# facebookresearch/nonrigid_nerf

Hardware: NVIDIA H100
Metric: rays/sec (64c+128f samples, 8x256 MLP), example_sequence training step (higher is better)
Workload: dtype f16 (tensor-core operands; f32 accumulate)

## Files before the change

### __graft_entry__.py

```python
import os
import subprocess
import sys

ROOT = os.path.dirname(os.path.abspath(__file__))
if ROOT not in sys.path:
    sys.path.insert(0, ROOT)


def build() -> None:
    subprocess.check_call(["make", "-j", str(min(8, os.cpu_count() or 1)), "-C", os.path.join(ROOT, "nonrigid_nerf_b200", "csrc")])
    subprocess.check_call(["make", "-C", os.path.join(ROOT, "tests", "cuda")])
    subprocess.check_call(["make", "-C", os.path.join(ROOT, "tests", "cuda"), "-f", "wgmma_rs_probe.mk"])
    import nonrigid_nerf_b200
    from nonrigid_nerf_b200 import _lib

    lib = _lib.load()
    assert lib.nrn_abi_version() == _lib.ABI_VERSION
    import oracle.nrnerf_oracle
    subprocess.check_call([sys.executable, os.path.join(ROOT, "oracle", "make_ref.py")])


def smoke() -> None:
    import numpy as np
    import torch

    import oracle.nrnerf_oracle as O
    from nonrigid_nerf_b200 import _lib, train as T
    from tests import helpers

    dev = "cuda:0"
    seed, n = 4242, 96
    coarse, fine, bender, (cp, fp, bp) = helpers.build_models(O, seed, dev)
    r = O.make_rays(seed, n)
    rnd = O.make_randomness(seed, n, 64, 64)
    lat = r["latents"].clone().to(dev).requires_grad_(True)
    kw = dict(network_query_fn=None, perturb=1.0, N_importance=64, network_fine=fine, N_samples=64, network_fn=coarse,
              ray_bender=bender, use_viewdirs=False, white_bkgd=False, raw_noise_std=1.0, ndc=False, lindisp=False,
              randomness=rnd)
    rgb, disp, acc, extras = T.render(r["rays_o"].to(dev), r["rays_d"].to(dev), chunk=32768, near=r["near"], far=r["far"],
                                      additional_pixel_information={"ray_bending_latents": lat}, detailed_output=True,
                                      retraw=True, **kw)
    tgt = r["target"].to(dev)
    loss = ((rgb - tgt) ** 2).mean() + ((extras["rgb0"] - tgt) ** 2).mean()
    loss.backward()
    _lib.device_error_check()

    cpo, fpo, bpo = O.clone_params(cp, True), O.clone_params(fp, True), O.clone_params(bp, True)
    ret = O.render_rays(cpo, fpo, bpo, r["rays_o"], r["rays_d"], r["near"], r["far"], r["latents"], 64, 64, perturb=True,
                        raw_noise_std=1.0, rnd=rnd)
    (((ret["rgb_map"] - r["target"]) ** 2).mean() + ((ret["rgb0"] - r["target"]) ** 2).mean()).backward()
    linf = float((rgb.detach().cpu() - ret["rgb_map"].detach()).abs().max())
    g, g_ref = fine.pts_linears[3].weight.grad.cpu(), fpo["pts_w"][3].grad
    rel = float((g - g_ref).norm() / g_ref.norm())
    print(f"smoke: rgb L-inf vs oracle {linf:.3e}; grad rel err (fine L3) {rel:.3e}; loss {float(loss):.5f}")
    assert np.isfinite(float(loss)) and linf <= 5e-4 and rel <= 3e-2, (linf, rel)


if __name__ == "__main__":
    build()
    if len(sys.argv) > 1 and sys.argv[1] == "smoke":
        smoke()
```

### nonrigid_nerf_b200/csrc/field_bwd.cu

```cuda
#include "field_mma.cuh"

namespace nrn {

namespace {

constexpr int kBwdStageLd = 66;
constexpr int kBwdRingStages = 4;
constexpr size_t kBwdSmemBytes = kHBytes + kBwdRingStages * kRingStageBytes + 2 * kWgRows * kBwdStageLd * sizeof(float) +
                                 sizeof(RingShared<kBwdRingStages>) + 64;
static_assert(kBwdSmemBytes <= 227 * 1024, "DGRAD kernel: dynamic shared memory per block");

static_assert(dgrad::step(dgrad::L6T) == dgrad::step(dgrad::L7T) && dgrad::step(dgrad::L5hT) == dgrad::step(dgrad::L7T) &&
              dgrad::step(dgrad::L4T) == dgrad::step(dgrad::L7T) && dgrad::step(dgrad::L3T) == dgrad::step(dgrad::L7T) &&
              dgrad::step(dgrad::L2T) == dgrad::step(dgrad::L7T) && dgrad::step(dgrad::L1T) == dgrad::step(dgrad::L7T),
              "step_at: one default shape; the consumers run L5h^T .. L1^T as one loop");
constexpr uint32_t kSlabA = 2 * dgrad::step(dgrad::L4T).k16 * kChunkBytes;

__device__ __forceinline__ Step step_at(int step) {
  switch (step) {
    case dgrad::HeadT: return step_imm<dgrad::HeadT>();
    case dgrad::L5eT: return step_imm<dgrad::L5eT>();
    case dgrad::L0T: return step_imm<dgrad::L0T>();
    case dgrad::B4T: return step_imm<dgrad::B4T>();
    case dgrad::B3T: return step_imm<dgrad::B3T>();
    case dgrad::B2T: return step_imm<dgrad::B2T>();
    case dgrad::B1T: return step_imm<dgrad::B1T>();
    case dgrad::B0T: return step_imm<dgrad::B0T>();
    default: return step_imm<dgrad::L7T>();
  }
}

__device__ __forceinline__ float clamp_h(float v) { return fminf(fmaxf(v, -65504.f), 65504.f); }

template <int NCOLS, int NR>
__device__ __forceinline__ void epi_mask_store(const float (&acc)[NR], const ReluMask<NCOLS>& m, uint8_t* img, int g) {
  const int r0 = g * kWgRows + acc_r0(), q = acc_q();
#pragma unroll
  for (int j = 0; j < NCOLS / 8; ++j) {
#pragma unroll
    for (int i = 0; i < 2; ++i) {
      const uint32_t g2 = pack_h2_sat(acc[4 * j + 2 * i], acc[4 * j + 2 * i + 1]);
      *reinterpret_cast<uint32_t*>(img + j * kChunkBytes + (r0 + 8 * i) * 16 + 4 * q) = m.apply(i, j, g2);
    }
  }
}

__device__ __forceinline__ float h_lo(uint32_t w) { return __half2float(__ushort_as_half(static_cast<unsigned short>(w & 0xffffu))); }
__device__ __forceinline__ float h_hi(uint32_t w) { return __half2float(__ushort_as_half(static_cast<unsigned short>(w >> 16))); }

__device__ __forceinline__ void pe_backward(const float* de, const uint8_t* __restrict__ e_row, float (&dx)[3]) {
  float e[64];
#pragma unroll
  for (int c = 0; c < 8; ++c) {
    const uint4 w = __ldg(reinterpret_cast<const uint4*>(e_row + c * kChunkBytes));
    e[c * 8 + 0] = h_lo(w.x); e[c * 8 + 1] = h_hi(w.x); e[c * 8 + 2] = h_lo(w.y); e[c * 8 + 3] = h_hi(w.y);
    e[c * 8 + 4] = h_lo(w.z); e[c * 8 + 5] = h_hi(w.z); e[c * 8 + 6] = h_lo(w.w); e[c * 8 + 7] = h_hi(w.w);
  }
#pragma unroll
  for (int d = 0; d < 3; ++d) {
    float acc = de[d];
#pragma unroll
    for (int k = 0; k < 10; ++k) {
      const float f = static_cast<float>(1 << k);
      const float s = e[3 + 6 * k + d], c = e[3 + 6 * k + 3 + d];
      acc += f * (de[3 + 6 * k + d] * c - de[3 + 6 * k + 3 + d] * s);
    }
    dx[d] += acc;
  }
}

}

template <bool HAS_BENDER>
__global__ void __launch_bounds__(kFwdThreads, 1) field_bwd_kernel(const FieldBwdParams p) {
  extern __shared__ __align__(1024) uint8_t smem[];
  uint8_t* act = smem;
  uint8_t* ring_buf = smem + kHBytes;
  float* stage_all = reinterpret_cast<float*>(ring_buf + kBwdRingStages * kRingStageBytes);
  auto* sh = reinterpret_cast<RingShared<kBwdRingStages>*>(stage_all + 2 * kWgRows * kBwdStageLd);

  const int warp = threadIdx.x >> 5;
  const int lane = threadIdx.x & 31;

  if (threadIdx.x == 0) sh->init();
  __syncthreads();
  const Waiter W{&sh->abort_flag, p.err};
  Ring<kBwdRingStages> ring{ring_buf, sh->w_full, sh->w_empty};

  if (warp >= 8) {
    setmaxnreg_dec<kProducerRegs>();
    if (warp == 8 && lane == 0) produce(p.nerf_wT, p.bend_wT, p.n_tiles, 0, HAS_BENDER ? dgrad::kCount : dgrad::B4T, dgrad::B4T, step_at, ring, W);
    return;
  }

  setmaxnreg_inc<kConsumerRegs>();
  const int g = warp >> 2;
  const int tw = threadIdx.x & 127;
  const bool row_thread = tw < kWgRows;
  const int bar = 1 + g;
  const bool wg_leader = tw == 0;
  const int row = g * kWgRows + tw;
  uint8_t* a_row = act + row * 16;
  const uint32_t a_base = smem_u32(act) + g * kWgRows * 16;
  auto a_slab = [&](uint32_t j) { return a_base + j * kSlabA; };
  float* stg = stage_all + g * kWgRows * kBwdStageLd;
  const float* my_stg = stg + tw * kBwdStageLd;

  const float scale = loss_scale(p.amax);
  const float inv_scale = 1.0f / scale;

  for (int tile = blockIdx.x; tile < p.n_tiles; tile += gridDim.x) {
    const long long pt = static_cast<long long>(tile) * kTileM + row;
    const bool valid = row_thread && pt < p.P;
    const uint8_t* st_tile = p.stash + static_cast<long long>(tile) * kStashTileBytes;
    const uint8_t* st = st_tile + row * 16;
    uint8_t* gs = p.gstash + static_cast<long long>(tile) * kGradTileBytes;
    const StashWriter<false> sw{gs, wg_leader, bar, g};
    const uint8_t* mk = p.relu_mask + static_cast<long long>(tile) * kMaskTileBytes;
    auto prefetch_e = [&]() {
      if (wg_leader) tma_prefetch_l2(st_tile + kStE.off, kEBytes);
    };
    sw.begin();
    if (row_thread) {
      float gr[4] = {0.f, 0.f, 0.f, 0.f};
      if (valid) {
        const float* q = p.d_raw + pt * p.out_ch;
#pragma unroll
        for (int c = 0; c < 4; ++c) gr[c] = clamp_h(__ldg(q + c) * scale);
      }
      *reinterpret_cast<uint4*>(a_row) = make_uint4(pack_h2(gr[0], gr[1]), pack_h2(gr[2], gr[3]), 0u, 0u);
      *reinterpret_cast<uint4*>(a_row + kChunkBytes) = make_uint4(0u, 0u, 0u, 0u);
    }
    sw.ready(kGsRaw, act);
    float dx[3] = {0.f, 0.f, 0.f};
#pragma unroll 1
    for (int s = 0; s < 3; ++s) {
      const Step st = step_at(dgrad::HeadT + s);
      Acc<dgrad::L7T> acc;
      ReluMask<kMaskHCols> m;
      m.load(mk + kMkH + (7 - s) * kMaskHBytes, g);
      wg_gemm<dgrad::step(dgrad::L7T).N>(acc, ring, st.nslabs, st.k16, a_slab, W, 300 + s);
      if (s == 2) prefetch_e();
      sw.begin();
      epi_mask_store<kMaskHCols>(acc, m, act, g);
      sw.ready({kGsY + (7 - s) * kHBytes, kHChunks}, act);
    }
    {
      Acc<dgrad::L5eT> acc;
      wg_gemm_step<dgrad::L5eT>(acc, ring, a_slab, W, 303);
      stage_cols<0, 8>(acc, stg, kBwdStageLd);
      wg_bar(bar);
      if (row_thread) pe_backward(my_stg, st + kStE.off, dx);
    }
#pragma unroll 1
    for (int s = 0; s < 5; ++s) {
      Acc<dgrad::L4T> acc;
      ReluMask<kMaskHCols> m;
      m.load(mk + kMkH + (4 - s) * kMaskHBytes, g);
      wg_gemm_step<dgrad::L4T>(acc, ring, a_slab, W, 304 + s);
      if (s == 4) prefetch_e();
      sw.begin();
      epi_mask_store<kMaskHCols>(acc, m, act, g);
      sw.ready({kGsY + (4 - s) * kHBytes, kHChunks}, act);
    }
    {
      Acc<dgrad::L0T> acc;
      wg_gemm_step<dgrad::L0T>(acc, ring, a_slab, W, 309);
      stage_cols<0, 8>(acc, stg, kBwdStageLd);
      wg_bar(bar);
      if (row_thread) pe_backward(my_stg, st + kStE.off, dx);
    }
    if (!HAS_BENDER) continue;

    float drpre = 0.f;
    sw.begin();
    if (row_thread) {
      float rig = 0.f, un[3] = {0.f, 0.f, 0.f}, dun[3], dm[3];
      float up_r = 0.f, up_u[3] = {0.f, 0.f, 0.f};
      if (valid) {
        rig = __ldg(p.rigidity + pt);
#pragma unroll
        for (int d = 0; d < 3; ++d) un[d] = __ldg(p.unmasked + pt * 3 + d);
        if (p.d_rigid_up) up_r = __ldg(p.d_rigid_up + pt) * scale;
        if (p.d_unmasked_up) {
#pragma unroll
          for (int d = 0; d < 3; ++d) up_u[d] = __ldg(p.d_unmasked_up + pt * 3 + d) * scale;
        }
      }
      float dr = up_r;
#pragma unroll
      for (int d = 0; d < 3; ++d) {
        dm[d] = p.use_scaling ? dx[d] * p.scaling : dx[d];
        dun[d] = rig * dm[d] + up_u[d];
        dr += un[d] * dm[d];
      }
      drpre = dr * 2.0f * rig * (1.0f - rig);
      if (p.use_cutoff && rig <= p.cutoff) drpre = 0.f;
      if (!valid) { dun[0] = dun[1] = dun[2] = 0.f; drpre = 0.f; }
      *reinterpret_cast<uint4*>(a_row) = make_uint4(pack_h2(clamp_h(dun[0]), clamp_h(dun[1])), pack_h2(clamp_h(dun[2]), 0.f), 0u, 0u);
      *reinterpret_cast<uint4*>(a_row + kChunkBytes) = make_uint4(0u, 0u, 0u, 0u);
    }
    sw.ready(kGsYb4, act);
    {
      Acc<dgrad::B4T> acc;
      ReluMask<kMkHb4.cols> m;
      m.load(mk + kMkHb4.off, g);
      wg_gemm_step<dgrad::B4T>(acc, ring, a_slab, W, 310);
      sw.begin();
      epi_mask_store<kMkHb4.cols>(acc, m, act, g);
      sw.ready(kGsYb3, act);
    }
    {
      Acc<dgrad::B3T> acc;
      ReluMask<kMkHb3.cols> m;
      m.load(mk + kMkHb3.off, g);
      wg_gemm_step<dgrad::B3T>(acc, ring, a_slab, W, 311);
      sw.begin();
      epi_mask_store<kMkHb3.cols>(acc, m, act, g);
      if (row_thread) {
        *reinterpret_cast<uint4*>(a_row + 8 * kChunkBytes) = make_uint4(pack_h2(clamp_h(drpre), 0.f), 0u, 0u, 0u);
        *reinterpret_cast<uint4*>(a_row + 9 * kChunkBytes) = make_uint4(0u, 0u, 0u, 0u);
      }
      sw.ready(kGsYb2, act);
    }
    {
      Acc<dgrad::B2T> acc;
      ReluMask<kMkHb2.cols> m;
      m.load(mk + kMkHb2.off, g);
      wg_gemm_step<dgrad::B2T>(acc, ring, a_slab, W, 312);
      sw.begin();
      epi_mask_store<kMkHb2.cols>(acc, m, act, g);
      sw.ready(kGsYb1, act);
      m.load(mk + kMkHb1.off, g);
      wg_gemm_step<dgrad::B1T>(acc, ring, a_slab, W, 313);
      sw.begin();
      epi_mask_store<kMkHb1.cols>(acc, m, act, g);
      sw.ready(kGsYb0, act);
    }
    {
      Acc<dgrad::B0T> acc;
      wg_gemm_step<dgrad::B0T>(acc, ring, a_slab, W, 314);
      stage_cols<0, 5>(acc, stg, kBwdStageLd);
      wg_bar(bar);
      if (row_thread) {
        float dl[32];
#pragma unroll
        for (int i = 0; i < 32; ++i) dl[i] = my_stg[6 + i] * inv_scale;
        const long long ray = valid ? pt / p.S : -1;
        const long long ray0 = __shfl_sync(0xffffffffu, ray, 0);
        if (__all_sync(0xffffffffu, ray == ray0 && valid)) {
          const float tot = warp_transpose_reduce(dl, lane);
          atomicAdd(p.d_latents + ray0 * kLatent + lane, tot);
        } else if (valid) {
#pragma unroll
          for (int i = 0; i < 32; ++i) atomicAdd(p.d_latents + ray * kLatent + i, dl[i]);
        }
      }
    }
  }
  if (wg_leader) tma_bulk_wait<0>();
}

cudaError_t launch_field_bwd(const FieldBwdParams& p, bool has_bender, int num_sms, cudaStream_t stream) {
  return launch_field(has_bender ? field_bwd_kernel<true> : field_bwd_kernel<false>, p, num_sms, kBwdSmemBytes, stream);
}

}
```

### nonrigid_nerf_b200/csrc/sm90_ptx.cuh

```cuda
#pragma once
#include <cuda_runtime.h>
#include <cuda_fp16.h>
#include <cuda_bf16.h>
#include <stdint.h>

namespace nrn {

__device__ __forceinline__ uint32_t smem_u32(const void* p) {
  return static_cast<uint32_t>(__cvta_generic_to_shared(p));
}

__device__ __forceinline__ void mbar_init(uint64_t* bar, uint32_t count) {
  asm volatile("mbarrier.init.shared::cta.b64 [%0], %1;\n" ::"r"(smem_u32(bar)), "r"(count) : "memory");
}
__device__ __forceinline__ void fence_mbar_init() {
  asm volatile("fence.mbarrier_init.release.cluster;\n" ::: "memory");
}
__device__ __forceinline__ void mbar_arrive(uint64_t* bar) {
  asm volatile("mbarrier.arrive.shared::cta.b64 _, [%0];\n" ::"r"(smem_u32(bar)) : "memory");
}
__device__ __forceinline__ void mbar_arrive_expect_tx(uint64_t* bar, uint32_t bytes) {
  asm volatile("mbarrier.arrive.expect_tx.shared::cta.b64 _, [%0], %1;\n" ::"r"(smem_u32(bar)), "r"(bytes)
               : "memory");
}
__device__ __forceinline__ bool mbar_try_wait(uint64_t* bar, uint32_t parity) {
  uint32_t ok;
  asm volatile(
      "{\n\t.reg .pred P;\n\t"
      "mbarrier.try_wait.parity.shared::cta.b64 P, [%1], %2;\n\t"
      "selp.b32 %0, 1, 0, P;\n\t}\n"
      : "=r"(ok)
      : "r"(smem_u32(bar)), "r"(parity)
      : "memory");
  return ok != 0;
}

__device__ __forceinline__ uint32_t cluster_ctarank() {
  uint32_t r;
  asm volatile("mov.u32 %0, %%cluster_ctarank;\n" : "=r"(r));
  return r;
}
__device__ __forceinline__ void cluster_sync() {
  asm volatile("barrier.cluster.arrive.release.aligned;\n\tbarrier.cluster.wait.acquire.aligned;\n" ::: "memory");
}
__device__ __forceinline__ uint32_t mapa_shared(const void* p, uint32_t rank) {
  uint32_t r;
  asm volatile("mapa.shared::cluster.u32 %0, %1, %2;\n" : "=r"(r) : "r"(smem_u32(p)), "r"(rank));
  return r;
}
__device__ __forceinline__ void mbar_arrive_cluster(uint32_t cluster_addr) {
  asm volatile("mbarrier.arrive.shared::cluster.b64 _, [%0];\n" ::"r"(cluster_addr) : "memory");
}
__device__ __forceinline__ void st_shared_cluster(uint32_t cluster_addr, int v) {
  asm volatile("st.relaxed.cluster.shared::cluster.u32 [%0], %1;\n" ::"r"(cluster_addr), "r"(v) : "memory");
}

__device__ __forceinline__ void fence_proxy_async_smem() {
  asm volatile("fence.proxy.async.shared::cta;\n" ::: "memory");
}

__device__ __forceinline__ void wg_bar(int id) { asm volatile("bar.sync %0, 128;" ::"r"(id) : "memory"); }

__device__ __forceinline__ void tma_bulk_g2s(void* smem_dst, const void* gmem_src, uint32_t bytes,
                                             uint64_t* bar) {
  asm volatile(
      "cp.async.bulk.shared::cluster.global.mbarrier::complete_tx::bytes [%0], [%1], %2, [%3];\n" ::"r"(
          smem_u32(smem_dst)),
      "l"(gmem_src), "r"(bytes), "r"(smem_u32(bar))
      : "memory");
}
__device__ __forceinline__ void tma_bulk_g2s_multicast(void* smem_dst, const void* gmem_src, uint32_t bytes, uint64_t* bar,
                                                       uint16_t cta_mask) {
  asm volatile(
      "cp.async.bulk.shared::cluster.global.mbarrier::complete_tx::bytes.multicast::cluster [%0], [%1], %2, [%3], %4;\n" ::"r"(
          smem_u32(smem_dst)),
      "l"(gmem_src), "r"(bytes), "r"(smem_u32(bar)), "h"(cta_mask)
      : "memory");
}
__device__ __forceinline__ void tma_bulk_s2g(void* gmem_dst, const void* smem_src, uint32_t bytes) {
  asm volatile("cp.async.bulk.global.shared::cta.bulk_group [%0], [%1], %2;\n" ::"l"(gmem_dst),
               "r"(smem_u32(smem_src)), "r"(bytes)
               : "memory");
}
__device__ __forceinline__ void tma_prefetch_l2(const void* gmem_src, uint32_t bytes) {
  asm volatile("cp.async.bulk.prefetch.L2.global [%0], %1;\n" ::"l"(gmem_src), "r"(bytes) : "memory");
}
__device__ __forceinline__ void tma_bulk_commit() { asm volatile("cp.async.bulk.commit_group;\n" ::: "memory"); }
template <int N>
__device__ __forceinline__ void tma_bulk_wait_read() {
  asm volatile("cp.async.bulk.wait_group.read %0;\n" ::"n"(N) : "memory");
}
template <int N>
__device__ __forceinline__ void tma_bulk_wait() {
  asm volatile("cp.async.bulk.wait_group %0;\n" ::"n"(N) : "memory");
}

template <int R>
__device__ __forceinline__ void setmaxnreg_dec() { asm volatile("setmaxnreg.dec.sync.aligned.u32 %0;\n" ::"n"(R)); }
template <int R>
__device__ __forceinline__ void setmaxnreg_inc() { asm volatile("setmaxnreg.inc.sync.aligned.u32 %0;\n" ::"n"(R)); }

__host__ __device__ __forceinline__ uint64_t gmma_desc(uint32_t saddr, uint32_t lbo_bytes, uint32_t sbo_bytes) {
  uint64_t d = 0;
  d |= static_cast<uint64_t>((saddr >> 4) & 0x3FFFu);
  d |= static_cast<uint64_t>((lbo_bytes >> 4) & 0x3FFFu) << 16;
  d |= static_cast<uint64_t>((sbo_bytes >> 4) & 0x3FFFu) << 32;
  return d;
}
__host__ __device__ __forceinline__ uint64_t gmma_desc_advance(uint64_t desc, uint32_t bytes) {
  return desc + static_cast<uint64_t>(bytes >> 4);
}

__device__ __forceinline__ void wgmma_fence() { asm volatile("wgmma.fence.sync.aligned;\n" ::: "memory"); }
__device__ __forceinline__ void wgmma_commit() { asm volatile("wgmma.commit_group.sync.aligned;\n" ::: "memory"); }
template <int NR>
__device__ __forceinline__ void acc_fence(float (&d)[NR]) {
#pragma unroll
  for (int i = 0; i < NR; ++i) asm volatile("" : "+f"(d[i])::"memory");
}
template <int N>
__device__ __forceinline__ void wgmma_wait() {
  asm volatile("wgmma.wait_group.sync.aligned %0;\n" ::"n"(N) : "memory");
}

template <int TA, int TB>
__device__ __forceinline__ void wgmma_m64n16(float (&d)[8], uint64_t adesc, uint64_t bdesc, uint32_t accumulate) {
  asm volatile(
      "{\n\t.reg .pred p;\n\t"
      "setp.ne.b32 p, %10, 0;\n\t"
      "wgmma.mma_async.sync.aligned.m64n16k16.f32.f16.f16 "
      "{%0, %1, %2, %3, %4, %5, %6, %7}, "
      "%8, %9, p, 1, 1, %11, %12;\n\t}\n"
      : "+f"(d[0]), "+f"(d[1]), "+f"(d[2]), "+f"(d[3]), "+f"(d[4]), "+f"(d[5]), "+f"(d[6]), "+f"(d[7])
      : "l"(adesc), "l"(bdesc), "r"(accumulate), "n"(TA), "n"(TB));
}

template <int TA, int TB>
__device__ __forceinline__ void wgmma_m64n48(float (&d)[24], uint64_t adesc, uint64_t bdesc, uint32_t accumulate) {
  asm volatile(
      "{\n\t.reg .pred p;\n\t"
      "setp.ne.b32 p, %26, 0;\n\t"
      "wgmma.mma_async.sync.aligned.m64n48k16.f32.f16.f16 "
      "{%0, %1, %2, %3, %4, %5, %6, %7, %8, %9, %10, %11, %12, %13, %14, %15, %16, %17, %18, %19, %20, %21, %22, %23}, "
      "%24, %25, p, 1, 1, %27, %28;\n\t}\n"
      : "+f"(d[0]), "+f"(d[1]), "+f"(d[2]), "+f"(d[3]), "+f"(d[4]), "+f"(d[5]), "+f"(d[6]), "+f"(d[7]), "+f"(d[8]), "+f"(d[9]), "+f"(d[10]), "+f"(d[11]), "+f"(d[12]), "+f"(d[13]), "+f"(d[14]), "+f"(d[15]), "+f"(d[16]), "+f"(d[17]), "+f"(d[18]), "+f"(d[19]), "+f"(d[20]), "+f"(d[21]), "+f"(d[22]), "+f"(d[23])
      : "l"(adesc), "l"(bdesc), "r"(accumulate), "n"(TA), "n"(TB));
}

template <int TA, int TB>
__device__ __forceinline__ void wgmma_m64n64(float (&d)[32], uint64_t adesc, uint64_t bdesc, uint32_t accumulate) {
  asm volatile(
      "{\n\t.reg .pred p;\n\t"
      "setp.ne.b32 p, %34, 0;\n\t"
      "wgmma.mma_async.sync.aligned.m64n64k16.f32.f16.f16 "
      "{%0, %1, %2, %3, %4, %5, %6, %7, %8, %9, %10, %11, %12, %13, %14, %15, %16, %17, %18, %19, %20, %21, %22, %23, %24, %25, %26, %27, %28, %29, %30, %31}, "
      "%32, %33, p, 1, 1, %35, %36;\n\t}\n"
      : "+f"(d[0]), "+f"(d[1]), "+f"(d[2]), "+f"(d[3]), "+f"(d[4]), "+f"(d[5]), "+f"(d[6]), "+f"(d[7]), "+f"(d[8]), "+f"(d[9]), "+f"(d[10]), "+f"(d[11]), "+f"(d[12]), "+f"(d[13]), "+f"(d[14]), "+f"(d[15]), "+f"(d[16]), "+f"(d[17]), "+f"(d[18]), "+f"(d[19]), "+f"(d[20]), "+f"(d[21]), "+f"(d[22]), "+f"(d[23]), "+f"(d[24]), "+f"(d[25]), "+f"(d[26]), "+f"(d[27]), "+f"(d[28]), "+f"(d[29]), "+f"(d[30]), "+f"(d[31])
      : "l"(adesc), "l"(bdesc), "r"(accumulate), "n"(TA), "n"(TB));
}

template <int TA, int TB>
__device__ __forceinline__ void wgmma_m64n80(float (&d)[40], uint64_t adesc, uint64_t bdesc, uint32_t accumulate) {
  asm volatile(
      "{\n\t.reg .pred p;\n\t"
      "setp.ne.b32 p, %42, 0;\n\t"
      "wgmma.mma_async.sync.aligned.m64n80k16.f32.f16.f16 "
      "{%0, %1, %2, %3, %4, %5, %6, %7, %8, %9, %10, %11, %12, %13, %14, %15, %16, %17, %18, %19, %20, %21, %22, %23, %24, %25, %26, %27, %28, %29, %30, %31, %32, %33, %34, %35, %36, %37, %38, %39}, "
      "%40, %41, p, 1, 1, %43, %44;\n\t}\n"
      : "+f"(d[0]), "+f"(d[1]), "+f"(d[2]), "+f"(d[3]), "+f"(d[4]), "+f"(d[5]), "+f"(d[6]), "+f"(d[7]), "+f"(d[8]), "+f"(d[9]), "+f"(d[10]), "+f"(d[11]), "+f"(d[12]), "+f"(d[13]), "+f"(d[14]), "+f"(d[15]), "+f"(d[16]), "+f"(d[17]), "+f"(d[18]), "+f"(d[19]), "+f"(d[20]), "+f"(d[21]), "+f"(d[22]), "+f"(d[23]), "+f"(d[24]), "+f"(d[25]), "+f"(d[26]), "+f"(d[27]), "+f"(d[28]), "+f"(d[29]), "+f"(d[30]), "+f"(d[31]), "+f"(d[32]), "+f"(d[33]), "+f"(d[34]), "+f"(d[35]), "+f"(d[36]), "+f"(d[37]), "+f"(d[38]), "+f"(d[39])
      : "l"(adesc), "l"(bdesc), "r"(accumulate), "n"(TA), "n"(TB));
}

template <int TA, int TB>
__device__ __forceinline__ void wgmma_m64n96(float (&d)[48], uint64_t adesc, uint64_t bdesc, uint32_t accumulate) {
  asm volatile(
      "{\n\t.reg .pred p;\n\t"
      "setp.ne.b32 p, %50, 0;\n\t"
      "wgmma.mma_async.sync.aligned.m64n96k16.f32.f16.f16 "
      "{%0, %1, %2, %3, %4, %5, %6, %7, %8, %9, %10, %11, %12, %13, %14, %15, %16, %17, %18, %19, %20, %21, %22, %23, %24, %25, %26, %27, %28, %29, %30, %31, %32, %33, %34, %35, %36, %37, %38, %39, %40, %41, %42, %43, %44, %45, %46, %47}, "
      "%48, %49, p, 1, 1, %51, %52;\n\t}\n"
      : "+f"(d[0]), "+f"(d[1]), "+f"(d[2]), "+f"(d[3]), "+f"(d[4]), "+f"(d[5]), "+f"(d[6]), "+f"(d[7]), "+f"(d[8]), "+f"(d[9]), "+f"(d[10]), "+f"(d[11]), "+f"(d[12]), "+f"(d[13]), "+f"(d[14]), "+f"(d[15]), "+f"(d[16]), "+f"(d[17]), "+f"(d[18]), "+f"(d[19]), "+f"(d[20]), "+f"(d[21]), "+f"(d[22]), "+f"(d[23]), "+f"(d[24]), "+f"(d[25]), "+f"(d[26]), "+f"(d[27]), "+f"(d[28]), "+f"(d[29]), "+f"(d[30]), "+f"(d[31]), "+f"(d[32]), "+f"(d[33]), "+f"(d[34]), "+f"(d[35]), "+f"(d[36]), "+f"(d[37]), "+f"(d[38]), "+f"(d[39]), "+f"(d[40]), "+f"(d[41]), "+f"(d[42]), "+f"(d[43]), "+f"(d[44]), "+f"(d[45]), "+f"(d[46]), "+f"(d[47])
      : "l"(adesc), "l"(bdesc), "r"(accumulate), "n"(TA), "n"(TB));
}

template <int TA, int TB>
__device__ __forceinline__ void wgmma_m64n256(float (&d)[128], uint64_t adesc, uint64_t bdesc, uint32_t accumulate) {
  asm volatile(
      "{\n\t.reg .pred p;\n\t"
      "setp.ne.b32 p, %130, 0;\n\t"
      "wgmma.mma_async.sync.aligned.m64n256k16.f32.f16.f16 "
      "{%0, %1, %2, %3, %4, %5, %6, %7, %8, %9, %10, %11, %12, %13, %14, %15, %16, %17, %18, %19, %20, %21, %22, %23, %24, %25, %26, %27, %28, %29, %30, %31, %32, %33, %34, %35, %36, %37, %38, %39, %40, %41, %42, %43, %44, %45, %46, %47, %48, %49, %50, %51, %52, %53, %54, %55, %56, %57, %58, %59, %60, %61, %62, %63, %64, %65, %66, %67, %68, %69, %70, %71, %72, %73, %74, %75, %76, %77, %78, %79, %80, %81, %82, %83, %84, %85, %86, %87, %88, %89, %90, %91, %92, %93, %94, %95, %96, %97, %98, %99, %100, %101, %102, %103, %104, %105, %106, %107, %108, %109, %110, %111, %112, %113, %114, %115, %116, %117, %118, %119, %120, %121, %122, %123, %124, %125, %126, %127}, "
      "%128, %129, p, 1, 1, %131, %132;\n\t}\n"
      : "+f"(d[0]), "+f"(d[1]), "+f"(d[2]), "+f"(d[3]), "+f"(d[4]), "+f"(d[5]), "+f"(d[6]), "+f"(d[7]), "+f"(d[8]), "+f"(d[9]), "+f"(d[10]), "+f"(d[11]), "+f"(d[12]), "+f"(d[13]), "+f"(d[14]), "+f"(d[15]), "+f"(d[16]), "+f"(d[17]), "+f"(d[18]), "+f"(d[19]), "+f"(d[20]), "+f"(d[21]), "+f"(d[22]), "+f"(d[23]), "+f"(d[24]), "+f"(d[25]), "+f"(d[26]), "+f"(d[27]), "+f"(d[28]), "+f"(d[29]), "+f"(d[30]), "+f"(d[31]), "+f"(d[32]), "+f"(d[33]), "+f"(d[34]), "+f"(d[35]), "+f"(d[36]), "+f"(d[37]), "+f"(d[38]), "+f"(d[39]), "+f"(d[40]), "+f"(d[41]), "+f"(d[42]), "+f"(d[43]), "+f"(d[44]), "+f"(d[45]), "+f"(d[46]), "+f"(d[47]), "+f"(d[48]), "+f"(d[49]), "+f"(d[50]), "+f"(d[51]), "+f"(d[52]), "+f"(d[53]), "+f"(d[54]), "+f"(d[55]), "+f"(d[56]), "+f"(d[57]), "+f"(d[58]), "+f"(d[59]), "+f"(d[60]), "+f"(d[61]), "+f"(d[62]), "+f"(d[63]), "+f"(d[64]), "+f"(d[65]), "+f"(d[66]), "+f"(d[67]), "+f"(d[68]), "+f"(d[69]), "+f"(d[70]), "+f"(d[71]), "+f"(d[72]), "+f"(d[73]), "+f"(d[74]), "+f"(d[75]), "+f"(d[76]), "+f"(d[77]), "+f"(d[78]), "+f"(d[79]), "+f"(d[80]), "+f"(d[81]), "+f"(d[82]), "+f"(d[83]), "+f"(d[84]), "+f"(d[85]), "+f"(d[86]), "+f"(d[87]), "+f"(d[88]), "+f"(d[89]), "+f"(d[90]), "+f"(d[91]), "+f"(d[92]), "+f"(d[93]), "+f"(d[94]), "+f"(d[95]), "+f"(d[96]), "+f"(d[97]), "+f"(d[98]), "+f"(d[99]), "+f"(d[100]), "+f"(d[101]), "+f"(d[102]), "+f"(d[103]), "+f"(d[104]), "+f"(d[105]), "+f"(d[106]), "+f"(d[107]), "+f"(d[108]), "+f"(d[109]), "+f"(d[110]), "+f"(d[111]), "+f"(d[112]), "+f"(d[113]), "+f"(d[114]), "+f"(d[115]), "+f"(d[116]), "+f"(d[117]), "+f"(d[118]), "+f"(d[119]), "+f"(d[120]), "+f"(d[121]), "+f"(d[122]), "+f"(d[123]), "+f"(d[124]), "+f"(d[125]), "+f"(d[126]), "+f"(d[127])
      : "l"(adesc), "l"(bdesc), "r"(accumulate), "n"(TA), "n"(TB));
}

template <int N, int TA, int TB>
__device__ __forceinline__ void wgmma(float (&d)[N / 2], uint64_t adesc, uint64_t bdesc, uint32_t accumulate) {
  static_assert(N == 16 || N == 48 || N == 64 || N == 80 || N == 96 || N == 256, "wgmma: N without a wrapper");
  if constexpr (N == 16) wgmma_m64n16<TA, TB>(d, adesc, bdesc, accumulate);
  else if constexpr (N == 48) wgmma_m64n48<TA, TB>(d, adesc, bdesc, accumulate);
  else if constexpr (N == 64) wgmma_m64n64<TA, TB>(d, adesc, bdesc, accumulate);
  else if constexpr (N == 80) wgmma_m64n80<TA, TB>(d, adesc, bdesc, accumulate);
  else if constexpr (N == 96) wgmma_m64n96<TA, TB>(d, adesc, bdesc, accumulate);
  else wgmma_m64n256<TA, TB>(d, adesc, bdesc, accumulate);
}

template <int TB>
__device__ __forceinline__ void wgmma_m64n16_rs(float (&d)[8], const uint32_t (&a)[4], uint64_t bdesc, uint32_t accumulate) {
  asm volatile(
      "{\n\t.reg .pred p;\n\t"
      "setp.ne.b32 p, %13, 0;\n\t"
      "wgmma.mma_async.sync.aligned.m64n16k16.f32.f16.f16 "
      "{%0, %1, %2, %3, %4, %5, %6, %7}, "
      "{%8, %9, %10, %11}, %12, p, 1, 1, %14;\n\t}\n"
      : "+f"(d[0]), "+f"(d[1]), "+f"(d[2]), "+f"(d[3]), "+f"(d[4]), "+f"(d[5]), "+f"(d[6]), "+f"(d[7])
      : "r"(a[0]), "r"(a[1]), "r"(a[2]), "r"(a[3]), "l"(bdesc), "r"(accumulate), "n"(TB));
}

template <int TB>
__device__ __forceinline__ void wgmma_m64n256_rs(float (&d)[128], const uint32_t (&a)[4], uint64_t bdesc, uint32_t accumulate) {
  asm volatile(
      "{\n\t.reg .pred p;\n\t"
      "setp.ne.b32 p, %133, 0;\n\t"
      "wgmma.mma_async.sync.aligned.m64n256k16.f32.f16.f16 "
      "{%0, %1, %2, %3, %4, %5, %6, %7, %8, %9, %10, %11, %12, %13, %14, %15, %16, %17, %18, %19, %20, %21, %22, %23, %24, %25, %26, %27, %28, %29, %30, %31, %32, %33, %34, %35, %36, %37, %38, %39, %40, %41, %42, %43, %44, %45, %46, %47, %48, %49, %50, %51, %52, %53, %54, %55, %56, %57, %58, %59, %60, %61, %62, %63, %64, %65, %66, %67, %68, %69, %70, %71, %72, %73, %74, %75, %76, %77, %78, %79, %80, %81, %82, %83, %84, %85, %86, %87, %88, %89, %90, %91, %92, %93, %94, %95, %96, %97, %98, %99, %100, %101, %102, %103, %104, %105, %106, %107, %108, %109, %110, %111, %112, %113, %114, %115, %116, %117, %118, %119, %120, %121, %122, %123, %124, %125, %126, %127}, "
      "{%128, %129, %130, %131}, %132, p, 1, 1, %134;\n\t}\n"
      : "+f"(d[0]), "+f"(d[1]), "+f"(d[2]), "+f"(d[3]), "+f"(d[4]), "+f"(d[5]), "+f"(d[6]), "+f"(d[7]), "+f"(d[8]), "+f"(d[9]), "+f"(d[10]), "+f"(d[11]), "+f"(d[12]), "+f"(d[13]), "+f"(d[14]), "+f"(d[15]), "+f"(d[16]), "+f"(d[17]), "+f"(d[18]), "+f"(d[19]), "+f"(d[20]), "+f"(d[21]), "+f"(d[22]), "+f"(d[23]), "+f"(d[24]), "+f"(d[25]), "+f"(d[26]), "+f"(d[27]), "+f"(d[28]), "+f"(d[29]), "+f"(d[30]), "+f"(d[31]), "+f"(d[32]), "+f"(d[33]), "+f"(d[34]), "+f"(d[35]), "+f"(d[36]), "+f"(d[37]), "+f"(d[38]), "+f"(d[39]), "+f"(d[40]), "+f"(d[41]), "+f"(d[42]), "+f"(d[43]), "+f"(d[44]), "+f"(d[45]), "+f"(d[46]), "+f"(d[47]), "+f"(d[48]), "+f"(d[49]), "+f"(d[50]), "+f"(d[51]), "+f"(d[52]), "+f"(d[53]), "+f"(d[54]), "+f"(d[55]), "+f"(d[56]), "+f"(d[57]), "+f"(d[58]), "+f"(d[59]), "+f"(d[60]), "+f"(d[61]), "+f"(d[62]), "+f"(d[63]), "+f"(d[64]), "+f"(d[65]), "+f"(d[66]), "+f"(d[67]), "+f"(d[68]), "+f"(d[69]), "+f"(d[70]), "+f"(d[71]), "+f"(d[72]), "+f"(d[73]), "+f"(d[74]), "+f"(d[75]), "+f"(d[76]), "+f"(d[77]), "+f"(d[78]), "+f"(d[79]), "+f"(d[80]), "+f"(d[81]), "+f"(d[82]), "+f"(d[83]), "+f"(d[84]), "+f"(d[85]), "+f"(d[86]), "+f"(d[87]), "+f"(d[88]), "+f"(d[89]), "+f"(d[90]), "+f"(d[91]), "+f"(d[92]), "+f"(d[93]), "+f"(d[94]), "+f"(d[95]), "+f"(d[96]), "+f"(d[97]), "+f"(d[98]), "+f"(d[99]), "+f"(d[100]), "+f"(d[101]), "+f"(d[102]), "+f"(d[103]), "+f"(d[104]), "+f"(d[105]), "+f"(d[106]), "+f"(d[107]), "+f"(d[108]), "+f"(d[109]), "+f"(d[110]), "+f"(d[111]), "+f"(d[112]), "+f"(d[113]), "+f"(d[114]), "+f"(d[115]), "+f"(d[116]), "+f"(d[117]), "+f"(d[118]), "+f"(d[119]), "+f"(d[120]), "+f"(d[121]), "+f"(d[122]), "+f"(d[123]), "+f"(d[124]), "+f"(d[125]), "+f"(d[126]), "+f"(d[127])
      : "r"(a[0]), "r"(a[1]), "r"(a[2]), "r"(a[3]), "l"(bdesc), "r"(accumulate), "n"(TB));
}

template <int N, int TB>
__device__ __forceinline__ void wgmma_rs(float (&d)[N / 2], const uint32_t (&a)[4], uint64_t bdesc, uint32_t accumulate) {
  static_assert(N == 16 || N == 256, "wgmma_rs: N without a wrapper");
  if constexpr (N == 16) wgmma_m64n16_rs<TB>(d, a, bdesc, accumulate);
  else wgmma_m64n256_rs<TB>(d, a, bdesc, accumulate);
}
template <int KF>
__device__ __forceinline__ uint32_t& frag_pair(uint32_t (&a)[KF][4], int j, int i) { return a[j >> 1][2 * (j & 1) + i]; }
template <int KF>
__device__ __forceinline__ void frag_fence(uint32_t (&a)[KF][4]) {
#pragma unroll
  for (int k = 0; k < KF; ++k)
#pragma unroll
    for (int i = 0; i < 4; ++i) asm volatile("" : "+r"(a[k][i])::"memory");
}

__device__ __forceinline__ uint32_t pack_h2(float a, float b) {
  __half2 h = __floats2half2_rn(a, b);
  return *reinterpret_cast<uint32_t*>(&h);
}
__device__ __forceinline__ uint32_t pack_h2_relu_sat(float a, float b) {
  uint32_t d;
  asm("cvt.rn.relu.satfinite.f16x2.f32 %0, %1, %2;" : "=r"(d) : "f"(b), "f"(a));
  return d;
}
__device__ __forceinline__ uint32_t pack_h2_sat(float a, float b) {
  uint32_t d;
  asm("cvt.rn.satfinite.f16x2.f32 %0, %1, %2;" : "=r"(d) : "f"(b), "f"(a));
  return d;
}
__device__ __forceinline__ uint32_t pack_bf2(float a, float b) {
  __nv_bfloat162 h = __floats2bfloat162_rn(a, b);
  return *reinterpret_cast<uint32_t*>(&h);
}

constexpr long long kWaitLimitCycles = 1ll << 28;

struct Waiter {
  int* s_abort;
  int* g_err;
  bool paired = false;
  uint32_t partner_abort = 0;
  __device__ __forceinline__ bool wait(uint64_t* bar, uint32_t parity, int code) const {
    if (mbar_try_wait(bar, parity)) return true;
    const long long t0 = clock64();
    while (!mbar_try_wait(bar, parity)) {
      if (*reinterpret_cast<volatile int*>(s_abort)) return false;
      if (clock64() - t0 > kWaitLimitCycles) {
        atomicExch(s_abort, code);
        if (paired) st_shared_cluster(partner_abort, code);
        atomicCAS(g_err, 0, code);
        return false;
      }
    }
    return true;
  }
};

template <int N>
__device__ __forceinline__ void transpose_reduce_step(float (&v)[32], int lane) {
  if constexpr (N > 1) {
    constexpr int off = N / 2;
    const bool upper = (lane & off) != 0;
#pragma unroll
    for (int i = 0; i < off; ++i) {
      const float lo = v[i], hi = v[i + off];
      v[i] = (upper ? hi : lo) + __shfl_xor_sync(0xffffffffu, upper ? lo : hi, off);
    }
    transpose_reduce_step<off>(v, lane);
  }
}

__device__ __forceinline__ float warp_transpose_reduce(float (&v)[32], int lane) {
  transpose_reduce_step<32>(v, lane);
  return v[0];
}

__device__ __forceinline__ float loss_scale(const float* amax_ptr) {
  float scale = 1.0f;
  const float amax = amax_ptr ? __ldg(amax_ptr) : 0.f;
  if (amax > 0.f && amax < 3.0e38f) {
    int e;
    frexpf(amax, &e);
    scale = ldexpf(1.0f, min(max(10 - e, -60), 60));
  }
  return scale;
}

}
```

Before: 424,100.

## Keep dgrad trunk activations in registers via wgmma RS operand, add ring stage

The backward dgrad trunk (head^T through L0^T) now feeds the next layer's MMA straight from register fragments (wgmma with A from registers) instead of writing the masked gradient to a shared activation slab and reading it back through descriptors. Gradient images still go to global scratch for the weight-gradient pass. The freed shared-memory activation area shrinks to the bender image size, which allows one more weight ring stage. A new m64n64 RS wrapper is added for the embedding-sized steps. The cost is much higher register pressure (128 accumulators plus 64 fragment registers per thread) and extra warpgroup barriers around staging.

After: 454,600 (median of 6 runs). +7.2%, better.

```diff
diff --git a/__graft_entry__.py b/__graft_entry__.py
--- a/__graft_entry__.py
+++ b/__graft_entry__.py
@@ -11,6 +11,7 @@
     subprocess.check_call(["make", "-j", str(min(8, os.cpu_count() or 1)), "-C", os.path.join(ROOT, "nonrigid_nerf_b200", "csrc")])
     subprocess.check_call(["make", "-C", os.path.join(ROOT, "tests", "cuda")])
     subprocess.check_call(["make", "-C", os.path.join(ROOT, "tests", "cuda"), "-f", "wgmma_rs_probe.mk"])
+    subprocess.check_call(["make", "-C", os.path.join(ROOT, "tests", "cuda"), "-f", "wgmma_rs64_probe.mk"])
     import nonrigid_nerf_b200
     from nonrigid_nerf_b200 import _lib
 
diff --git a/nonrigid_nerf_b200/csrc/field_bwd.cu b/nonrigid_nerf_b200/csrc/field_bwd.cu
--- a/nonrigid_nerf_b200/csrc/field_bwd.cu
+++ b/nonrigid_nerf_b200/csrc/field_bwd.cu
@@ -5,8 +5,11 @@
 namespace {
 
 constexpr int kBwdStageLd = 66;
-constexpr int kBwdRingStages = 4;
-constexpr size_t kBwdSmemBytes = kHBytes + kBwdRingStages * kRingStageBytes + 2 * kWgRows * kBwdStageLd * sizeof(float) +
+constexpr int kBwdActBytes = kGsYb1.chunks * kChunkBytes;
+static_assert(kGsYb4.chunks <= kGsYb1.chunks && kGsYb3.chunks <= kGsYb1.chunks && kGsYb2.chunks <= kGsYb1.chunks &&
+              kGsYb0.chunks <= kGsYb1.chunks, "bender gradient images fit act");
+constexpr int kBwdRingStages = 5;
+constexpr size_t kBwdSmemBytes = kBwdActBytes + kBwdRingStages * kRingStageBytes + 2 * kWgRows * kBwdStageLd * sizeof(float) +
                                  sizeof(RingShared<kBwdRingStages>) + 64;
 static_assert(kBwdSmemBytes <= 227 * 1024, "DGRAD kernel: dynamic shared memory per block");
 
@@ -45,6 +48,20 @@
   }
 }
 
+__device__ __forceinline__ void epi_mask_frag(const float (&acc)[kMaskHCols / 2], const ReluMask<kMaskHCols>& m,
+                                              uint32_t (&a)[kMaskHCols / 16][4], uint8_t* gs_img, int g) {
+  const int r0 = g * kWgRows + acc_r0(), q = acc_q();
+#pragma unroll
+  for (int j = 0; j < kMaskHCols / 8; ++j) {
+#pragma unroll
+    for (int i = 0; i < 2; ++i) {
+      const uint32_t g2 = m.apply(i, j, pack_h2_sat(acc[4 * j + 2 * i], acc[4 * j + 2 * i + 1]));
+      frag_pair(a, j, i) = g2;
+      *reinterpret_cast<uint32_t*>(gs_img + j * kChunkBytes + (r0 + 8 * i) * 16 + 4 * q) = g2;
+    }
+  }
+}
+
 __device__ __forceinline__ float h_lo(uint32_t w) { return __half2float(__ushort_as_half(static_cast<unsigned short>(w & 0xffffu))); }
 __device__ __forceinline__ float h_hi(uint32_t w) { return __half2float(__ushort_as_half(static_cast<unsigned short>(w >> 16))); }
 
@@ -75,7 +92,7 @@
 __global__ void __launch_bounds__(kFwdThreads, 1) field_bwd_kernel(const FieldBwdParams p) {
   extern __shared__ __align__(1024) uint8_t smem[];
   uint8_t* act = smem;
-  uint8_t* ring_buf = smem + kHBytes;
+  uint8_t* ring_buf = smem + kBwdActBytes;
   float* stage_all = reinterpret_cast<float*>(ring_buf + kBwdRingStages * kRingStageBytes);
   auto* sh = reinterpret_cast<RingShared<kBwdRingStages>*>(stage_all + 2 * kWgRows * kBwdStageLd);
 
@@ -120,34 +137,51 @@
     auto prefetch_e = [&]() {
       if (wg_leader) tma_prefetch_l2(st_tile + kStE.off, kEBytes);
     };
-    sw.begin();
-    if (row_thread) {
-      float gr[4] = {0.f, 0.f, 0.f, 0.f};
-      if (valid) {
-        const float* q = p.d_raw + pt * p.out_ch;
-#pragma unroll
-        for (int c = 0; c < 4; ++c) gr[c] = clamp_h(__ldg(q + c) * scale);
-      }
-      *reinterpret_cast<uint4*>(a_row) = make_uint4(pack_h2(gr[0], gr[1]), pack_h2(gr[2], gr[3]), 0u, 0u);
-      *reinterpret_cast<uint4*>(a_row + kChunkBytes) = make_uint4(0u, 0u, 0u, 0u);
-    }
-    sw.ready(kGsRaw, act);
+    constexpr Step kTrunk = dgrad::step(dgrad::L7T), kEmb = dgrad::step(dgrad::L5eT);
+    static_assert(dgrad::step(dgrad::L0T) == kEmb && kEmb.nslabs == 1 && kEmb.k16 == kMaskHCols / 16, "L5e^T, L0^T: one slab, K = 256");
+    uint32_t h[kMaskHCols / 16][4];
+    {
+      static_assert(dgrad::step(dgrad::HeadT).N == kTrunk.N && dgrad::step(dgrad::HeadT).nslabs == 1 &&
+                    dgrad::step(dgrad::HeadT).k16 == 1 && kGsRaw.chunks == 2, "head^T: one K = 16 MMA");
+      const int r0 = g * kWgRows + acc_r0(), q = acc_q();
+      uint32_t a[1][4];
+#pragma unroll
+      for (int i = 0; i < 2; ++i) {
+        const long long pti = static_cast<long long>(tile) * kTileM + r0 + 8 * i;
+        float g0 = 0.f, g1 = 0.f;
+        if (q < 2 && pti < p.P) {
+          const float* src = p.d_raw + pti * p.out_ch + 2 * q;
+          g0 = clamp_h(__ldg(src) * scale);
+          g1 = clamp_h(__ldg(src + 1) * scale);
+        }
+        a[0][i] = q < 2 ? pack_h2(g0, g1) : 0u;
+        a[0][2 + i] = 0u;
+      }
+#pragma unroll
+      for (int j = 0; j < 2; ++j)
+#pragma unroll
+        for (int i = 0; i < 2; ++i)
+          *reinterpret_cast<uint32_t*>(gs + kGsRaw.off + j * kChunkBytes + (r0 + 8 * i) * 16 + 4 * q) = frag_pair(a, j, i);
+      Acc<dgrad::HeadT> acc;
+      ReluMask<kMaskHCols> m;
+      m.load(mk + kMkH + 7 * kMaskHBytes, g);
+      wg_gemm_rs<kTrunk.N, 1>(acc, a, ring, false, 0u, W, 300);
+      epi_mask_frag(acc, m, h, gs + kGsY + 7 * kHBytes, g);
+    }
     float dx[3] = {0.f, 0.f, 0.f};
 #pragma unroll 1
-    for (int s = 0; s < 3; ++s) {
-      const Step st = step_at(dgrad::HeadT + s);
+    for (int s = 0; s < 2; ++s) {
       Acc<dgrad::L7T> acc;
       ReluMask<kMaskHCols> m;
-      m.load(mk + kMkH + (7 - s) * kMaskHBytes, g);
-      wg_gemm<dgrad::step(dgrad::L7T).N>(acc, ring, st.nslabs, st.k16, a_slab, W, 300 + s);
-      if (s == 2) prefetch_e();
-      sw.begin();
-      epi_mask_store<kMaskHCols>(acc, m, act, g);
-      sw.ready({kGsY + (7 - s) * kHBytes, kHChunks}, act);
+      m.load(mk + kMkH + (6 - s) * kMaskHBytes, g);
+      wg_gemm_rs<kTrunk.N, kTrunk.k16>(acc, h, ring, false, 0u, W, 301 + s);
+      if (s == 1) prefetch_e();
+      epi_mask_frag(acc, m, h, gs + kGsY + (6 - s) * kHBytes, g);
     }
     {
       Acc<dgrad::L5eT> acc;
-      wg_gemm_step<dgrad::L5eT>(acc, ring, a_slab, W, 303);
+      wg_gemm_rs<kEmb.N, kEmb.k16>(acc, h, ring, false, 0u, W, 303);
+      wg_bar(bar);
       stage_cols<0, 8>(acc, stg, kBwdStageLd);
       wg_bar(bar);
       if (row_thread) pe_backward(my_stg, st + kStE.off, dx);
@@ -157,15 +191,14 @@
       Acc<dgrad::L4T> acc;
       ReluMask<kMaskHCols> m;
       m.load(mk + kMkH + (4 - s) * kMaskHBytes, g);
-      wg_gemm_step<dgrad::L4T>(acc, ring, a_slab, W, 304 + s);
+      wg_gemm_rs<kTrunk.N, kTrunk.k16>(acc, h, ring, false, 0u, W, 304 + s);
       if (s == 4) prefetch_e();
-      sw.begin();
-      epi_mask_store<kMaskHCols>(acc, m, act, g);
-      sw.ready({kGsY + (4 - s) * kHBytes, kHChunks}, act);
+      epi_mask_frag(acc, m, h, gs + kGsY + (4 - s) * kHBytes, g);
     }
     {
       Acc<dgrad::L0T> acc;
-      wg_gemm_step<dgrad::L0T>(acc, ring, a_slab, W, 309);
+      wg_gemm_rs<kEmb.N, kEmb.k16>(acc, h, ring, false, 0u, W, 309);
+      wg_bar(bar);
       stage_cols<0, 8>(acc, stg, kBwdStageLd);
       wg_bar(bar);
       if (row_thread) pe_backward(my_stg, st + kStE.off, dx);
diff --git a/nonrigid_nerf_b200/csrc/sm90_ptx.cuh b/nonrigid_nerf_b200/csrc/sm90_ptx.cuh
--- a/nonrigid_nerf_b200/csrc/sm90_ptx.cuh
+++ b/nonrigid_nerf_b200/csrc/sm90_ptx.cuh
@@ -219,6 +219,18 @@
 }
 
 template <int TB>
+__device__ __forceinline__ void wgmma_m64n64_rs(float (&d)[32], const uint32_t (&a)[4], uint64_t bdesc, uint32_t accumulate) {
+  asm volatile(
+      "{\n\t.reg .pred p;\n\t"
+      "setp.ne.b32 p, %37, 0;\n\t"
+      "wgmma.mma_async.sync.aligned.m64n64k16.f32.f16.f16 "
+      "{%0, %1, %2, %3, %4, %5, %6, %7, %8, %9, %10, %11, %12, %13, %14, %15, %16, %17, %18, %19, %20, %21, %22, %23, %24, %25, %26, %27, %28, %29, %30, %31}, "
+      "{%32, %33, %34, %35}, %36, p, 1, 1, %38;\n\t}\n"
+      : "+f"(d[0]), "+f"(d[1]), "+f"(d[2]), "+f"(d[3]), "+f"(d[4]), "+f"(d[5]), "+f"(d[6]), "+f"(d[7]), "+f"(d[8]), "+f"(d[9]), "+f"(d[10]), "+f"(d[11]), "+f"(d[12]), "+f"(d[13]), "+f"(d[14]), "+f"(d[15]), "+f"(d[16]), "+f"(d[17]), "+f"(d[18]), "+f"(d[19]), "+f"(d[20]), "+f"(d[21]), "+f"(d[22]), "+f"(d[23]), "+f"(d[24]), "+f"(d[25]), "+f"(d[26]), "+f"(d[27]), "+f"(d[28]), "+f"(d[29]), "+f"(d[30]), "+f"(d[31])
+      : "r"(a[0]), "r"(a[1]), "r"(a[2]), "r"(a[3]), "l"(bdesc), "r"(accumulate), "n"(TB));
+}
+
+template <int TB>
 __device__ __forceinline__ void wgmma_m64n256_rs(float (&d)[128], const uint32_t (&a)[4], uint64_t bdesc, uint32_t accumulate) {
   asm volatile(
       "{\n\t.reg .pred p;\n\t"
@@ -232,8 +244,9 @@
 
 template <int N, int TB>
 __device__ __forceinline__ void wgmma_rs(float (&d)[N / 2], const uint32_t (&a)[4], uint64_t bdesc, uint32_t accumulate) {
-  static_assert(N == 16 || N == 256, "wgmma_rs: N without a wrapper");
+  static_assert(N == 16 || N == 64 || N == 256, "wgmma_rs: N without a wrapper");
   if constexpr (N == 16) wgmma_m64n16_rs<TB>(d, a, bdesc, accumulate);
+  else if constexpr (N == 64) wgmma_m64n64_rs<TB>(d, a, bdesc, accumulate);
   else wgmma_m64n256_rs<TB>(d, a, bdesc, accumulate);
 }
 template <int KF>
```
